# The-Learning-And-Vision-Atelier-LAVA/BUFFER

Measured on AMD Instinct MI355X. Metric: registration pairs/sec, higher is better.
Workload: dtype f32

## Files before the change

buffer_amd/_lib.py:

```python
import ctypes as C
import os

_HERE = os.path.dirname(os.path.abspath(__file__))
LIB_PATH = os.environ.get("BUF_LIB_PATH") or os.path.join(_HERE, "libbuffer_hip.so")

BUF_OK = 0


class BufferHipError(RuntimeError):
    pass


class buf_grid_t(C.Structure):
    _fields_ = [
        ("ws", C.c_void_p), ("ws_bytes", C.c_size_t),
        ("ns", C.c_int), ("nb", C.c_int),
        ("cells_per_elem", C.c_int64),
        ("radius", C.c_float),
        ("supports", C.c_void_p),
        ("desc", C.c_void_p), ("s_off", C.c_void_p), ("table", C.c_void_p),
        ("sorted", C.c_void_p), ("order", C.c_void_p), ("scan_tmp", C.c_void_p),
    ]


# ... 16 lines not shown
    "buf_grid_subsample_ws_bytes": (_sz, [_i, _i, _i64, _i]),
    "buf_grid_subsample_batch": (_i, [_vp, _i, _vp, _i, _f, _i, _vp, _i, _vp, _vp, _vp, _vp, _i64, _vp, _sz, _vp]),
    "buf_fps_ws_bytes": (_sz, [_i, _i]),
    "buf_fps": (_i, [_vp, _i, _i, _i, _vp, _vp, _sz, _vp]),
    "buf_gather": (_i, [_vp, _vp, _i, _i, _i, _i, _vp, _vp]),
    "buf_group": (_i, [_vp, _vp, _i, _i, _i, _i, _i, _vp, _vp]),
    "buf_ball_query": (_i, [_vp, _vp, _i, _i, _i, _f, _i, _vp, _vp]),
    "buf_three_nn": (_i, [_vp, _vp, _i, _i, _i, _vp, _vp, _vp]),
    "buf_select_patches": (_i, [_vp, _vp, _i, _i, _f, _i, _vp, _vp]),
    "buf_select_patches_batched_ws_bytes": (_sz, [_i, _i]),
    "buf_select_patches_batched": (_i, [_vp, _vp, _i, _vp, _i, _f, _i, _vp, _vp, _sz, _vp]),
    "buf_permute_clouds": (_i, [_vp, _vp, _vp, _i, _vp, _vp]),
    "buf_compact_ws_bytes": (_sz, [_i]),
    "buf_compact_greater": (_i, [_vp, _i, _i, _f, _vp, _vp, _vp, _sz, _vp]),
    "buf_knn_ws_bytes": (_sz, [_i, _i, _i]),
    "buf_knn1_ws_bytes": (_sz, [_i, _i, _i]),
    "buf_knn": (_i, [_vp, _vp, _i, _i, _i, _i, _i, _vp, _vp, _vp, _sz, _vp]),
    "buf_fps_ragged": (_i, [_vp, _vp, _i, _i, _vp, _vp, _sz, _vp]),
    "buf_svd3x3_batched": (_i, [_vp, _i, _vp, _vp, _vp, _vp]),
    "buf_vn_gather_block": (_i, [_vp, _vp, _vp, _vp, _i, _i, _i, _i, _i, _i, _f, _vp, _vp, _vp, _vp, _f, _vp, _vp]),
    "buf_vn_gather_pre_ws_bytes": (_sz, [_i, _i]),
    "buf_vn_gather_block_pre": (_i, [_vp, _vp, _vp, _vp, _i, _i, _i, _i, _i, _f, _vp, _vp, _vp, _vp, _f, _vp, _vp, _sz, _vp]),
    "buf_vn_pointwise": (_i, [_vp, _vp, _i, _i, _i, _vp, _i, _i, _i, _vp, _vp, _vp, _vp, _f, _vp, _vp, _vp]),
    "buf_gather_max": (_i, [_vp, _vp, _i, _i, _i, _i, _vp, _vp]),
    "buf_vn_std": (_i, [_vp, _vp, _i, _i, _vp, _vp]),
    "buf_score_head_ws_bytes": (_sz, [_i, _i]),
    "buf_score_head": (_i, [_vp, _i, _vp, _i, _vp, _vp, _vp, _vp, _f, _vp, _vp, _vp, _vp, _f, _vp, _vp, _vp, _vp, _vp, _i, _vp, _vp, _i, _f,
                            _vp, _vp, _sz, _vp]),
    "buf_patch_voxelize_ws_bytes": (_sz, [_i]),
    "buf_patch_voxelize": (_i, [_vp, _vp, _i, _i, _f, _vp, _i, _i, _vp, _f, _i, _vp, _vp, _vp, _vp, _vp, _vp, _vp,
                                _vp, _vp, _sz, _vp]),
    "buf_cylindrical_net_wg": (_i, [_vp, _i, _vp, _vp, _vp, _vp, _vp, _vp, _vp]),
    "buf_cylindrical_net_wg_supports": (_i, [_vp, _vp]),
    "buf_cylindrical_net_split_safe": (_i, [_vp, _i, _vp, _vp, _vp, _vp, _vp, _vp, _vp, _vp, _vp, _vp, _vp, _vp]),
    "buf_cost_volume_net_split_safe": (_i, [_vp, _vp, _i, _vp, _vp, _i, _vp, _vp, _vp, _vp, _vp, _vp, _vp, _vp]),
    "buf_cylindrical_net_split": (_i, [_vp, _i, _vp, _vp, _vp, _vp, _vp, _vp, _vp, _vp]),
    "buf_cylindrical_net_split_head": (_i, [_vp, _i, _vp, _vp, _vp, _vp, _vp, _vp, _vp, _vp, _vp, _vp]),
    "buf_split_gemm_count": (C.c_longlong, [_i, _i, _i, _i]),
    "buf_split_tile_gemm": (_i, [_vp, _i, _i, _i, _i, _vp]),
    "buf_cost_volume_net_split": (_i, [_vp, _vp, _i, _vp, _vp, _vp, _vp, _vp]),
    "buf_cost_volume_net_split_gather": (_i, [_vp, _i, _vp, _vp, _i, _vp, _vp, _vp, _vp, _vp]),
    "buf_split_filter_count": (C.c_longlong, [_i, _i]),
    "buf_split_tile_filters": (_i, [_vp, _i, _i, _vp]),
    "buf_winograd_tile_weights": (_i, [_vp, _i, _i, _vp]),
    "buf_winograd_f24_tile_weights": (_i, [_vp, _i, _i, _vp]),
    "buf_winograd_group": (_i, [_i, _i]),
    "buf_cost_winograd_group": (_i, [_i]),
    "buf_winograd_tile_filters": (_i, [_vp, _i, _i, _i, _i, _vp]),
    "buf_voxel_downsample_ws_bytes": (_sz, [_i, _i64]),
    "buf_voxel_downsample": (_i, [_vp, _vp, _i, _i, C.c_double, _vp, _vp, _vp, _i64, _vp, _sz, _vp]),
    "buf_voxel_downsample_batch_ws_bytes": (_sz, [_i, _i, _i64]),
    "buf_voxel_downsample_batch": (_i, [_vp, _i, _i, _vp, _i, C.c_double, _vp, _vp, _i64, _vp, _sz, _vp]),
    "buf_knn_normals": (_i, [_vp, _i, _vp, _i, _vp, _i, _i, _vp, _i, _vp, _vp, _vp]),
    "buf_icp_ws_bytes": (_sz, [_i, _i, _i, _i]),
    "buf_icp_batched": (_i, [_vp, _vp, _vp, _vp, _vp, _i, _i, _f, _vp, _i, C.c_double, C.c_double, _vp, _vp, _vp, _vp, _vp,
                             _vp, _sz, _vp]),
    "buf_pair_stats_ws_bytes": (_sz, [_i, _i, _i, _i, _i64]),
    "buf_pair_stats": (_i, [_vp, _vp, _i, _vp, _vp, _i, _vp, _f, _i64, _vp, _vp, _vp, _vp, _sz, _vp]),
    "buf_match_metrics": (_i, [_vp, _vp, _vp, _i, _i, _vp, _vp, _f, _f, _f, _vp, _vp, _vp]),
    "buf_row_linear": (_i, [_vp, _i, _i, _i, _vp, _vp, _i, _vp, _vp]),
    "buf_segment_instance_norm_ws_bytes": (_sz, [_i, _i]),
    "buf_segment_instance_norm": (_i, [_vp, _i, _i, _vp, _i, _f, _vp, _vp, _sz, _vp]),
    "buf_descriptor_head": (_i, [_vp, _i, _vp, _vp, _vp, _vp]),
    "buf_cost_volume_net": (_i, [_vp, _vp, _i, _vp, _vp, _vp, _vp]),
    "buf_cost_volume_net_gather": (_i, [_vp, _i, _vp, _vp, _i, _vp, _vp, _vp, _vp]),
    "buf_hypotheses_score": (_i, [_vp, _vp, _vp, _vp, _vp, _i, _i, _f, _vp, _vp, _vp, _vp, _vp, _vp]),
# ... 36 lines not shown
```

buffer_amd/csrc/buffer_hip.hip:

```cpp
#include <stdlib.h>
#include "core.hip"
#include "radius.hip"
#include "icp.hip"
#include "pairstats.hip"
#include "metrics.hip"
#include "subsample.hip"
#include "pointops.hip"
#include "vn.hip"
#include "voxelize.hip"
#include "registration.hip"
#include "convnet.hip"
#include "convnet_h3.hip"
#include "costnet_h3.hip"
#include "preprocess.hip"
#include "convnet_wg.hip"
#include "convnet_w24.hip"
#include "costnet.hip"
#include "split_safe.hip"
```

buffer_amd/csrc/convnet_w24.hip:

```cpp
#include "common.h"

#define W24_WSTRIDE 768
#define W24_SET_F22(CIN) (16 * 128 * (CIN))

__device__ __forceinline__ void w24_tile(int li, int& ty, int& tx)
{
    const bool last = li == 15;
    ty = last ? 3 : li / 5;
    tx = last ? 4 : li - 5 * ty;
}

__device__ __forceinline__ unsigned w24_row_addr(unsigned act_addr, int a, int li, int lk)
{
    int ty, tx;
    w24_tile(li, ty, tx);
    const int row = 2 * ty - 1 + a;
    return act_addr + 4u * (unsigned)(lk * WG_CS + ((row >= 0 && row <= 6) ? row * WG_ROW + 4 * tx : WG_ZERO));
}

struct W24AddrPark { float a[4]; };
__device__ __forceinline__ void w24_park_addresses(const float* act, int li, int lk, W24AddrPark& pk)
{
    const unsigned act_addr = (unsigned)(size_t)(__attribute__((address_space(3))) const float*)act;
#pragma unroll
// ... 58 lines not shown
        const unsigned adv = more ? 4u * WG_KSTEP : 0u;
        __builtin_amdgcn_sched_barrier(0);
#pragma unroll
        for (int s = 0; s < 4; s++) {
            if (s < 2) W24_LOAD(D[s & 1], P0, P1, (s + 2) * WG_KSTEP)
            else {
                if (s == 2) { P0 += adv; P1 += adv; }
                if constexpr (INEXT >= 0) {
                    unsigned q0 = more ? P0 : RA[A1N], q1 = more ? P1 : RA[A2N];
                    W24_LOAD(D[s & 1], q0, q1, (s - 2) * WG_KSTEP)
                } else
                    W24_LOAD(D[s & 1], P0, P1, (s - 2) * WG_KSTEP)
            }
            __builtin_amdgcn_sched_barrier(0);
#pragma unroll
            for (int n = 0; n < 2; n++)
#pragma unroll
                for (int j = 0; j < 6; j++)
                    acc[n][j] = __builtin_amdgcn_mfma_f32_16x16x4f32(W24_U(n, s & 1, j), V[s & 1][j], acc[n][j], 0, 0, 0);
            __builtin_amdgcn_sched_barrier(0);
            W24_XFORM((s + 1) & 1)
#pragma unroll
            for (int n = 0; n < 2; n++) {
                const unsigned o = s < 2 ? wcur + (s + 2) * W24_WSTRIDE : wn + (s - 2) * W24_WSTRIDE;
                W4[n][s & 1] = wg_ldw(rs, o + n * 256, lofs4);
                W2[n][s & 1] = w24_ldw2(rs, o + 512 + n * 128, lofs2);
            }
            __builtin_amdgcn_sched_barrier(0);
        }
    }
#undef W24_XFORM
}

__device__ __forceinline__ void w24_round(unsigned (&RA)[4], __amdgpu_buffer_rsrc_t rs, unsigned wp, unsigned wp_after, unsigned lofs4, unsigned lofs2,
                                          int niter, unsigned pstride, const float* __restrict__ bias_lane, wgf4 (&W4)[2][2], wgf2 (&W2)[2][2],
                                          wgf4 (&Y)[2][2][4])
{
    using std::integral_constant;
    wgf2 D[2][6];
    wgf4 bv[2];
#pragma unroll
    for (int n = 0; n < 2; n++) bv[n] = *reinterpret_cast<const wgf4*>(bias_lane + n * 16);
    wgf4 acc[2][6];
    float zero = 0.f;
    asm volatile("" : "+v"(zero));
#pragma unroll
    for (int n = 0; n < 2; n++)
#pragma unroll
        for (int j = 0; j < 6; j++) acc[n][j] = (wgf4){ zero, zero, zero, zero };
    auto run = [&](auto ic) __attribute__((always_inline)) {
        constexpr int I = decltype(ic)::value;
        constexpr int INEXT = I == 3 ? 0 : I + 1;
        if constexpr (I == 1) {
#pragma unroll
            for (int n = 0; n < 2; n++) acc[n][1] += bv[n];
        }
        constexpr int ICHAIN = (INEXT != 0 && wg_chains(I)) ? INEXT : -1;
        w24_pass<I, wg_chains(I - 1), ICHAIN>(RA, rs, wp + I * pstride, INEXT == 0 ? wp_after : wp + (I + 1) * pstride, lofs4, lofs2, niter, W4, W2, acc, D);
        __builtin_amdgcn_sched_barrier(0);
#pragma unroll
        for (int n = 0; n < 2; n++) {
            wgf4 f[4];
#pragma unroll
            for (int r = 0; r < 4; r++) {
                const float p = acc[n][1][r] + acc[n][2][r], q = acc[n][1][r] - acc[n][2][r];
                const float t = acc[n][3][r] + acc[n][4][r], d = acc[n][3][r] - acc[n][4][r];
                f[0][r] = acc[n][0][r] + p + t;
                f[1][r] = __builtin_fmaf(2.f, d, q);
                f[2][r] = __builtin_fmaf(4.f, t, p);
                f[3][r] = __builtin_fmaf(8.f, d, q) + acc[n][5][r];
            }
#pragma unroll
            for (int v = 0; v < 4; v++) {
                if constexpr (I == 0) Y[n][1][v] = f[v];
                else if constexpr (I == 1) {
#pragma unroll
                    for (int r = 0; r < 4; r++) Y[n][1][v][r] = __builtin_fmaf(2.f, f[v][r], -Y[n][1][v][r]);
                }
                else if constexpr (I == 2) Y[n][0][v] = f[v];
                else Y[n][1][v] -= f[v];
                if constexpr (I == 2) asm volatile("" : "+v"(Y[n][0][v]));
                else asm volatile("" : "+v"(Y[n][1][v]));
            }
        }
    };
    run(integral_constant<int, 0>{});
    run(integral_constant<int, 1>{});
    run(integral_constant<int, 2>{});
    run(integral_constant<int, 3>{});
}

__device__ __forceinline__ void w24_round_direct(unsigned row5, __amdgpu_buffer_rsrc_t rs, unsigned wp, unsigned lofs, int niter, unsigned pstride,
                                                 const float* __restrict__ bias_lane, wgf4 (&W4)[2][2], wgf4 (&Y)[2])
{
    constexpr int wstride = W24_WSTRIDE;
    wgf4 Wr[3][2][2];
#pragma unroll
    for (int n = 0; n < 2; n++)
#pragma unroll
        for (int k = 0; k < 2; k++) {
            Wr[0][n][k] = W4[n][k];
            Wr[1][n][k] = wg_ldw(rs, wp + pstride + n * 256 + k * wstride, lofs);
            Wr[2][n][k] = wg_ldw(rs, wp + 2 * pstride + n * 256 + k * wstride, lofs);
        }
    float X[2][6];
    unsigned pa = row5;
    WG_LOADD(X[0], pa, 0)
    WG_LOADD(X[1], pa, WG_KSTEP)
    wgf4 acc[2][3];
    float zero = 0.f;
    asm volatile("" : "+v"(zero));
#pragma unroll
    for (int n = 0; n < 2; n++) {
        acc[n][0] = (wgf4){ zero, zero, zero, zero };
        acc[n][1] = (wgf4){ zero, zero, zero, zero };
        acc[n][2] = *reinterpret_cast<const wgf4*>(bias_lane + n * 16);
    }
    float G[2][6];
#define W24_TAPS(SLOT)                                                                                    \
    _Pragma("unroll") for (int n = 0; n < 2; n++) {                                                       \
        const wgf4 u0_ = Wr[0][n][SLOT], u1_ = Wr[1][n][SLOT], u2_ = Wr[2][n][SLOT];                      \
        const float d1_ = wg_sub(u1_[1], u2_[1]), d2_ = wg_sub(u1_[2], u2_[2]);                           \
        G[n][0] = u0_[0]; G[n][1] = wg_sub(u0_[1], u0_[2]); G[n][2] = u0_[3];                             \
        G[n][3] = wg_sub(u1_[0], u2_[0]); G[n][4] = wg_sub(d1_, d2_); G[n][5] = wg_sub(u1_[3], u2_[3]);   \
    }
#define W24_RELOAD(SLOT, OFS)                                                                             \
    _Pragma("unroll") for (int n = 0; n < 2; n++)                                                         \
        _Pragma("unroll") for (int blk = 0; blk < 3; blk++) Wr[blk][n][SLOT] = wg_ldw(rs, (OFS) + blk * pstride + n * 256, lofs);
    W24_TAPS(0)
    W24_RELOAD(0, wp + 2 * wstride)
#pragma unroll 1
    for (int it = 0; it < niter; it++) {
        const bool more = it + 1 < niter;
        const unsigned wcur = wp + 4 * it * wstride;
        const unsigned wn = more ? wcur + 4 * wstride : wp;
        const unsigned adv = more ? 4u * WG_KSTEP : 0u;
        __builtin_amdgcn_sched_barrier(0);
#pragma unroll
        for (int s = 0; s < 4; s++) {
#pragma unroll
            for (int b = 0; b < 3; b++)
#pragma unroll
                for (int a = 0; a < 2; a++)
#pragma unroll
                    for (int n = 0; n < 2; n++)
                        acc[n][b] = __builtin_amdgcn_mfma_f32_16x16x4f32(G[n][a * 3 + b], X[s & 1][a * 3 + b], acc[n][b], 0, 0, 0);
            __builtin_amdgcn_sched_barrier(0);
            if (s < 2) WG_LOADD(X[s & 1], pa, (s + 2) * WG_KSTEP)
            else {
// ... 129 lines not shown
__global__ void __launch_bounds__(WG_THREADS, 2) k_cyl_net_w24_rerun(const float* __restrict__ x, CylWgParams P, float* __restrict__ y)
{
    extern __shared__ float lds[];
    if (P.only_if[blockIdx.x] == 0) return;
    cyl_net_w24_body(x, P, y, lds);
}

extern "C" int buf_winograd_f24_tile_weights(const float* w_host, int cout, int cin, float* out_host)
{
    BUF_REQUIRE(w_host && out_host, BUF_EINVAL, "buf_winograd_f24_tile_weights: null argument");
    BUF_REQUIRE(cout > 0 && cin > 0 && cout % 32 == 0 && cin % 4 == 0, BUF_EINVAL, "buf_winograd_f24_tile_weights: widths %d -> %d", cin, cout);
    static const double G2[4][3] = { { 1, 0, 0 }, { .5, .5, .5 }, { .5, -.5, .5 }, { 0, 0, 1 } };
    const double s6 = 1.0 / 6, s12 = 1.0 / 12, s24 = 1.0 / 24;
    const double G4[6][3] = { { .25, 0, 0 }, { -s6, -s6, -s6 }, { -s6, s6, -s6 }, { s24, s12, s6 }, { s24, -s12, s6 }, { 0, 0, 1 } };
    const int k4 = cin / 4;
    for (int o = 0; o < cout; o++)
        for (int c = 0; c < cin; c++) {
            const float* g = w_host + ((size_t)o * cin + c) * 9;
            const int n = o / 16, lane = (c % 4) * 16 + o % 16;
            for (int i = 0; i < 4; i++) {
                float* blk = out_host + (((size_t)(n / 2) * 4 + i) * k4 + c / 4) * W24_WSTRIDE;
                for (int j = 0; j < 6; j++) {
                    double u = 0;
                    for (int a = 0; a < 3; a++)
                        for (int b = 0; b < 3; b++) u += G2[i][a] * (double)g[3 * a + b] * G4[j][b];
                    if (j == 3 || j == 4) blk[512 + (n % 2) * 128 + lane * 2 + (j - 3)] = (float)u;
                    else blk[(n % 2) * 256 + lane * 4 + (j == 5 ? 3 : j)] = (float)u;
                }
            }
        }
    return BUF_OK;
}

static int w24_launch(const float* x, int npatch, CylWgParams P, float* y, void* stream)
{
    for (int l = 0; l < WG_LAYERS; l++) {
        const bool flag = (P.relu[l] & WG_F24_FLAG) != 0;
        BUF_REQUIRE(P.relu[l] >= 0 && P.relu[l] <= (WG_F24_FLAG | 1), BUF_EINVAL, "buf_cylindrical_net_wg: layer %d has relu flags %d", l, P.relu[l]);
        BUF_REQUIRE(flag == (P.cout[l] == 128), BUF_EINVAL,
                    "buf_cylindrical_net_wg: the F(2x4) flag goes on every layer with 128 output channels and on no other (layer %d: %d -> %d, flags %d)",
                    l, P.cin[l], P.cout[l], P.relu[l]);
        if (flag) P.wt[l] += W24_SET_F22(P.cin[l]);
        P.relu[l] &= 1;
    }
    size_t lds = sizeof(float) * WG_BUF;
    static LdsGrant grant, grant_rerun;
    if (int rc = P.only_if ? grant_dynamic_lds((const void*)k_cyl_net_w24_rerun, lds, grant_rerun) : grant_dynamic_lds((const void*)k_cyl_net_w24, lds, grant)) return rc;
    double macs = 0;
    for (int l = 0; l < WG_LAYERS; l++) macs += 9.0 * P.cin[l] * P.cout[l];
    TimedSpan span;
    bool timed = !P.only_if && timing_begin((hipStream_t)stream, &span, 2.0 * 140 * macs * npatch, BUF_TIMED_CYL_NET);
    if (P.only_if) k_cyl_net_w24_rerun<<<npatch, WG_THREADS, lds, (hipStream_t)stream>>>(x, P, y);
    else k_cyl_net_w24<<<npatch, WG_THREADS, lds, (hipStream_t)stream>>>(x, P, y);
    if (timed) timing_end((hipStream_t)stream, &span);
    BUF_LAUNCH_CHECK();
    return BUF_OK;
}
```

buffer_amd/csrc/convnet_wg.hip:

```cpp
#include "common.h"
#include <type_traits>

#define WG_CS 160
#define WG_ROW 22
#define WG_ZERO 154
#define WG_MAXC 128
#define WG_LAYERS 8
#define WG_THREADS 256
#define WG_BUF (WG_MAXC * WG_CS)
#define WG_KSTEP (16 * WG_CS)
#define WG_BLOCKS 16

typedef float wgf4 __attribute__((ext_vector_type(4)));
typedef float wgf2 __attribute__((ext_vector_type(2)));
typedef const __attribute__((address_space(3))) wgf2* wg_lds_f2;

struct CylWgParams {
    const float* wt[WG_LAYERS];
    const float* bias[WG_LAYERS];
    int cin[WG_LAYERS], cout[WG_LAYERS], relu[WG_LAYERS];
    const int* only_if;
#ifdef WG_STAMP
    long long* stamps;
#endif
// ... 588 lines not shown
extern "C" int buf_winograd_tile_weights(const float* w_host, int cout, int cin, float* out_host)
{
    BUF_REQUIRE(cout > 0 && cin > 0 && cout % 16 == 0 && cin % 4 == 0, BUF_EINVAL, "buf_winograd_tile_weights: widths %d -> %d", cin, cout);
    return buf_winograd_tile_filters(w_host, cout, cin, wg_group(cin, cout), WG_BLOCKS / 4, out_host);
}

extern "C" int buf_winograd_group(int cin, int cout) { return wg_group(cin, cout); }

static int wg_check_widths(const int* cin, const int* cout)
{
    for (int l = 0; l < WG_LAYERS; l++) {
        const int ci = cin[l], co = cout[l];
        BUF_REQUIRE(ci > 0 && ci % 16 == 0 && ci <= WG_MAXC && (co == 32 || co == 64 || co == 128), BUF_EINVAL,
                    "buf_cylindrical_net_wg: layer %d has unsupported widths %d -> %d", l, ci, co);
        BUF_REQUIRE(co != 128 || ci % 32 == 0, BUF_EINVAL,
                    "buf_cylindrical_net_wg: layer %d has unsupported widths %d -> %d (128 output channels need Cin %% 32 == 0)", l, ci, co);
        BUF_REQUIRE(co != 32 || (ci % 32 == 0 && ci <= 64), BUF_EINVAL,
                    "buf_cylindrical_net_wg: layer %d has unsupported widths %d -> %d (32 output channels need Cin = 32 or 64)", l, ci, co);
        BUF_REQUIRE(l == 0 || ci == cout[l - 1], BUF_EINVAL, "buf_cylindrical_net_wg: layer %d width mismatch", l);
        BUF_REQUIRE(l == 0 || cout[l - 1] != 32 || co == 32, BUF_EINVAL,
                    "buf_cylindrical_net_wg: layer %d has unsupported widths %d -> %d (only 32-output layers may follow a 32-output layer)", l, ci, co);
    }
    BUF_REQUIRE(cout[WG_LAYERS - 1] == 32, BUF_EINVAL, "buf_cylindrical_net_wg: the last layer must have 32 channels");
    return BUF_OK;
}

extern "C" int buf_cylindrical_net_wg_supports(const int* cin_host, const int* cout_host)
{
    BUF_REQUIRE(cin_host && cout_host, BUF_EINVAL, "buf_cylindrical_net_wg_supports: null argument");
    return wg_check_widths(cin_host, cout_host);
}

#define WG_F24_FLAG BUF_CYL_F24
static inline bool wg_f24_flagged(int relu) { return relu == WG_F24_FLAG || relu == (WG_F24_FLAG | 1); }
static int w24_launch(const float* x, int npatch, CylWgParams P, float* y, void* stream);

static int wg_launch(const float* x, int npatch, const float* const* wt_host, const float* const* bias_host, const int* cin_host,
                     const int* cout_host, const int* relu_host, float* y, const int* only_if, void* stream)
{
    BUF_REQUIRE(npatch >= 0, BUF_EINVAL, "buf_cylindrical_net_wg: npatch=%d", npatch);
    if (npatch == 0) return BUF_OK;
    BUF_REQUIRE(x && y && wt_host && bias_host && cin_host && cout_host && relu_host, BUF_EINVAL, "buf_cylindrical_net_wg: null argument");
    CylWgParams P;
    for (int l = 0; l < WG_LAYERS; l++) {
        P.wt[l] = wt_host[l]; P.bias[l] = bias_host[l];
        P.cin[l] = cin_host[l]; P.cout[l] = cout_host[l]; P.relu[l] = relu_host[l];
        BUF_REQUIRE(P.wt[l] && P.bias[l], BUF_EINVAL, "buf_cylindrical_net_wg: null weights for layer %d", l);
    }
    if (int rc = wg_check_widths(P.cin, P.cout)) return rc;
    P.only_if = only_if;
    for (int l = 0; l < WG_LAYERS; l++)
        if (wg_f24_flagged(relu_host[l])) return w24_launch(x, npatch, P, y, stream);
    size_t lds = sizeof(float) * WG_BUF;
    static LdsGrant grant, grant_rerun;
    if (int rc = only_if ? grant_dynamic_lds((const void*)k_cyl_net_wg_rerun, lds, grant_rerun) : grant_dynamic_lds((const void*)k_cyl_net_wg, lds, grant)) return rc;
    double macs = 0;
    for (int l = 0; l < WG_LAYERS; l++) macs += 9.0 * P.cin[l] * P.cout[l];
    TimedSpan span;
    bool timed = !only_if && timing_begin((hipStream_t)stream, &span, 2.0 * 140 * macs * npatch, BUF_TIMED_CYL_NET);
#ifdef WG_STAMP
    BUF_CHECK_HIP(hipMalloc(&P.stamps, (size_t)npatch * (4 * 20 + 4) * sizeof(long long)));
#endif
    if (only_if) k_cyl_net_wg_rerun<<<npatch, WG_THREADS, lds, (hipStream_t)stream>>>(x, P, y);
    else k_cyl_net_wg<<<npatch, WG_THREADS, lds, (hipStream_t)stream>>>(x, P, y);
    if (timed) timing_end((hipStream_t)stream, &span);
    BUF_LAUNCH_CHECK();
#ifdef WG_STAMP
// ... 35 lines not shown
```

buffer_amd/csrc/core.hip:

```cpp
#include "common.h"
#include <stdarg.h>

static thread_local char g_err[512] = "";

void buf_set_error(const char* fmt, ...)
{
    va_list ap;
    va_start(ap, fmt);
    vsnprintf(g_err, sizeof(g_err), fmt, ap);
    va_end(ap);
}

extern "C" const char* buf_last_error(void) { return g_err; }
extern "C" int buf_version(void) { return 600; }

#include <mutex>
#include <vector>
struct TimedSpan { hipEvent_t a, b; double bytes; int id; };
static std::mutex g_time_mu;
static std::vector<TimedSpan> g_spans;
static int g_timing_on = 0;

extern "C" void buf_timing_enable(int on) { std::lock_guard<std::mutex> l(g_time_mu); g_timing_on = on; }

static bool timing_begin(hipStream_t s, TimedSpan* sp, double bytes, int id = BUF_TIMED_GRID_QUERY)
{
    if (!g_timing_on) return false;
    sp->id = id;
    if (hipEventCreate(&sp->a) != hipSuccess || hipEventCreate(&sp->b) != hipSuccess) return false;
    sp->bytes = bytes;
    (void)hipEventRecord(sp->a, s);
    return true;
}

static void timing_end(hipStream_t s, TimedSpan* sp)
{
    (void)hipEventRecord(sp->b, s);
    std::lock_guard<std::mutex> l(g_time_mu);
    g_spans.push_back(*sp);
}

extern "C" long long buf_timing_collect_kernel(int id, double* total_ms, double* total_work)
{
    std::lock_guard<std::mutex> l(g_time_mu);
    double ms = 0, by = 0;
    long long n = 0;
    std::vector<TimedSpan> keep;
// ... 223 lines not shown
```

buffer_amd/csrc/split_safe.hip:

```cpp
#include "common.h"

extern "C" int buf_cylindrical_net_split_safe(const float* x, int npatch, const void* const* wt_split_host, const float* const* wt_wg_host,
                                              const float* const* bias_host, const int* cin_host, const int* cout_host, const int* relu_host,
                                              const float* head_params, float* y_or_equi, float* desc, int* status_dev, int* flags_ws,
                                              void* stream)
{
    BUF_REQUIRE(npatch >= 0, BUF_EINVAL, "buf_cylindrical_net_split_safe: npatch=%d", npatch);
    if (npatch == 0) return BUF_OK;
    BUF_REQUIRE(x && y_or_equi && flags_ws && wt_split_host && wt_wg_host && bias_host && cin_host && cout_host && relu_host, BUF_EINVAL,
                "buf_cylindrical_net_split_safe: null argument");
    BUF_REQUIRE(!head_params || desc, BUF_EINVAL, "buf_cylindrical_net_split_safe: head without desc");
    if (int rc = buf_cylindrical_net_wg_supports(cin_host, cout_host)) return rc;
    hipStream_t s = (hipStream_t)stream;
    BUF_CHECK_HIP(hipMemsetAsync(flags_ws, 0, sizeof(int) * (size_t)npatch, s));
    int relu_split[WG_LAYERS];
    for (int l = 0; l < WG_LAYERS; l++) relu_split[l] = wg_f24_flagged(relu_host[l]) ? (relu_host[l] & 1) : relu_host[l];
    int rc = h3_launch(x, npatch, wt_split_host, bias_host, cin_host, cout_host, relu_split, head_params ? nullptr : y_or_equi, head_params,
                       desc, head_params ? y_or_equi : nullptr, status_dev, stream, flags_ws);
    if (rc) return rc;
    rc = wg_launch(x, npatch, wt_wg_host, bias_host, cin_host, cout_host, relu_host, y_or_equi, flags_ws, stream);
    if (rc) return rc;
    if (head_params) {
        k_desc_head_masked<<<npatch, DH_THREADS, 0, s>>>(y_or_equi, head_params, desc, y_or_equi, flags_ws);
        BUF_LAUNCH_CHECK();
    }
    return BUF_OK;
}

extern "C" int buf_cost_volume_net_split_safe(const float* s_eq, const float* t_eq, int ele_n, const long long* s_rows, const long long* t_rows,
                                              int m, const void* const* wt_split_host, const float* const* bias_split_host,
                                              const float* const* wt_f32_host, const float* const* bias_f32_host, float* ind_out,
                                              int* status_dev, int* flags_ws, void* stream)
{
    BUF_REQUIRE(m >= 0, BUF_EINVAL, "buf_cost_volume_net_split_safe: m=%d", m);
    if (m == 0) return BUF_OK;
    BUF_REQUIRE(s_eq && t_eq && wt_split_host && bias_split_host && wt_f32_host && bias_f32_host && ind_out && flags_ws, BUF_EINVAL,
                "buf_cost_volume_net_split_safe: null argument");
    BUF_REQUIRE((s_rows == nullptr) == (t_rows == nullptr), BUF_EINVAL, "buf_cost_volume_net_split_safe: one row list without the other");
    BUF_REQUIRE(!s_rows || ele_n == 7, BUF_EINVAL, "buf_cost_volume_net_split_safe: ele_n=%d (the kernels are built for ele_n = 7)", ele_n);
    hipStream_t s = (hipStream_t)stream;
    BUF_CHECK_HIP(hipMemsetAsync(flags_ws, 0, sizeof(int) * (size_t)m, s));
    int rc = cost_net_h3_launch(s_eq, t_eq, m, wt_split_host, bias_split_host, s_rows, t_rows, ele_n, ind_out, status_dev, stream,
                                "buf_cost_volume_net_split_safe", flags_ws);
    if (rc) return rc;
    return cost_net_launch(s_eq, t_eq, m, wt_f32_host, bias_f32_host, s_rows, t_rows, ele_n, ind_out, stream, "buf_cost_volume_net_split_safe", flags_ws);
// ... 2 lines not shown
```

buffer_amd/ops.py:

```python
import ctypes as C
import time
import os
import numpy as np
import torch

from . import _lib
from ._lib import buf_grid_t, check


def _stream():
    return C.c_void_p(torch.cuda.current_stream().cuda_stream)


def _dev(t, dtype, what):
    if not isinstance(t, torch.Tensor) or not t.is_cuda:
        raise _lib.BufferHipError(f"{what}: expected a tensor in device memory (buffer_amd has no CPU path)")
    if t.dtype != dtype:
        t = t.to(dtype)
    return t.contiguous()


def _ptr(t):
    return C.c_void_p(t.data_ptr()) if t is not None else C.c_void_p(0)

# ... 560 lines not shown
    G5 = np.concatenate([G, [[0, 1, 0]]])
    U = np.einsum('ia,ocab,jb->ijoc', G5, np.asarray(w, np.float64), G)
    U = U[:blocks].reshape(blocks, 4, cout // (16 * ng), ng, 16, cin // 4, 4)
    return np.ascontiguousarray(np.transpose(U, (2, 0, 5, 3, 6, 4, 1)), dtype=np.float32).reshape(-1)


def winograd_f24_tile_weights(w):
    cout, cin = w.shape[0], w.shape[1]
    assert cin % 4 == 0 and cout % 32 == 0
    U = winograd_f24_filters(w)
    U = U.reshape(4, 6, cout // 32, 2, 16, cin // 4, 4)
    U = np.transpose(U, (2, 0, 5, 3, 6, 4, 1))
    lead = U.shape[:3]
    wide = U[..., [0, 1, 2, 5]].reshape(*lead, 512)
    narrow = U[..., [3, 4]].reshape(*lead, 256)
    return np.ascontiguousarray(np.concatenate([wide, narrow], axis=-1), dtype=np.float32).reshape(-1)


F24_G2 = np.array([[1, 0, 0], [.5, .5, .5], [.5, -.5, .5], [0, 0, 1]], np.float64)
F24_G4 = np.array([[.25, 0, 0], [-1 / 6, -1 / 6, -1 / 6], [-1 / 6, 1 / 6, -1 / 6], [1 / 24, 1 / 12, 1 / 6], [1 / 24, -1 / 12, 1 / 6], [0, 0, 1]],
                  np.float64)


def winograd_f24_filters(w):
    w64 = np.asarray(w, np.float64)
    U = np.zeros((4, 6) + w64.shape[:2], np.float64)
    for a in range(3):
        for b in range(3):
            U += (F24_G2[:, a][:, None, None, None] * w64[None, None, :, :, a, b]) * F24_G4[:, b][None, :, None, None]
    return U


F24_FLAG = 2


def cyl_layer_filters(w):
    wt = winograd_tile_weights(w)
    if w.shape[0] != 128:
        return wt, 0
    return np.concatenate([wt, winograd_f24_tile_weights(w)]), F24_FLAG


class CylindricalNet:

    def __init__(self, layers, device, f24=True):
        self.wt, self.bias, self.cin, self.cout, self.relu = [], [], [], [], []
        self.entry = "buf_cylindrical_net_wg"
        flags = []
        for w, b, relu in layers:
            cout, cin = w.shape[0], w.shape[1]
            wt, flag = cyl_layer_filters(w) if f24 else (winograd_tile_weights(w), 0)
            flags.append(flag)
            self.wt.append(torch.from_numpy(wt).to(device))
            self.bias.append(torch.from_numpy(np.ascontiguousarray(b, dtype=np.float32)).to(device))
            self.cin.append(cin); self.cout.append(cout); self.relu.append(1 if relu else 0)
        n = len(layers)
        self._wp = (C.c_void_p * n)(*[t.data_ptr() for t in self.wt])
        self._bp = (C.c_void_p * n)(*[t.data_ptr() for t in self.bias])
        self._ci = (C.c_int * n)(*self.cin)
        self._co = (C.c_int * n)(*self.cout)
        self._re = (C.c_int * n)(*[r | f for r, f in zip(self.relu, flags)])

    def __call__(self, x):
        L = _lib.lib()
        x = x.contiguous()
        P = x.shape[0]
        y = torch.empty((P, self.cout[-1], 7, 20), dtype=torch.float32, device=x.device)
        check(L.buf_cylindrical_net_wg(_ptr(x), P, self._wp, self._bp, self._ci, self._co, self._re, _ptr(y), _stream()), self.entry)
        return y


def split_tile_filters(w):
    L = _lib.lib()
    w = np.ascontiguousarray(w, dtype=np.float32)
    cout, cin = w.shape[0], w.shape[1]
    out = np.empty(L.buf_split_filter_count(cout, cin), dtype=np.uint16)
    check(L.buf_split_tile_filters(w.ctypes.data, cout, cin, out.ctypes.data), "buf_split_tile_filters")
    return out


class CylindricalNetSplit:

    def __init__(self, layers, device):
        self.wt, self.bias, self.cin, self.cout, self.relu = [], [], [], [], []
        self.entry = "buf_cylindrical_net_split"
        for w, b, relu in layers:
            cout, cin = w.shape[0], w.shape[1]
            self.wt.append(torch.from_numpy(split_tile_filters(w).view(np.int16)).to(device))
            self.bias.append(torch.from_numpy(np.ascontiguousarray(b, dtype=np.float32)).to(device))
            self.cin.append(cin); self.cout.append(cout); self.relu.append(1 if relu else 0)
        n = len(layers)
        self.status = torch.zeros(1, dtype=torch.int32, device=device)
        self._wp = (C.c_void_p * n)(*[t.data_ptr() for t in self.wt])
        self._bp = (C.c_void_p * n)(*[t.data_ptr() for t in self.bias])
        self._ci = (C.c_int * n)(*self.cin)
        self._co = (C.c_int * n)(*self.cout)
        self._re = (C.c_int * n)(*self.relu)
        self.last_flags = None
        self.safe = n == 8 and _lib.lib().buf_cylindrical_net_wg_supports(self._ci, self._co) == 0 and not os.environ.get('BUF_SPLIT_UNSAFE')
        if self.safe:
            tiled = [cyl_layer_filters(w) for w, _, _ in layers]
            self.wt_wg = [torch.from_numpy(wt).to(device) for wt, _ in tiled]
            self._wwp = (C.c_void_p * n)(*[t.data_ptr() for t in self.wt_wg])
            self._re_safe = (C.c_int * n)(*[r | f for r, (_, f) in zip(self.relu, tiled)])

    def _safe_call(self, x, head):
        L = _lib.lib()
        x = x.contiguous()
        P = x.shape[0]
        out = torch.empty((P, self.cout[-1], 7, 20), dtype=torch.float32, device=x.device)
        desc = torch.empty((P, 32), dtype=torch.float32, device=x.device) if head is not None else None
        self.last_flags = torch.empty((max(P, 1),), dtype=torch.int32, device=x.device)
        check(L.buf_cylindrical_net_split_safe(_ptr(x), P, self._wp, self._wwp, self._bp, self._ci, self._co, self._re_safe,
                                               _ptr(head.params) if head is not None else None, _ptr(out), _ptr(desc), _ptr(self.status),
                                               _ptr(self.last_flags), _stream()), "buf_cylindrical_net_split_safe")
        return (desc, out) if head is not None else out

    def __call__(self, x):
        if self.safe:
            return self._safe_call(x, None)
        L = _lib.lib()
        x = x.contiguous()
        P = x.shape[0]
        y = torch.empty((P, self.cout[-1], 7, 20), dtype=torch.float32, device=x.device)
        check(L.buf_cylindrical_net_split(_ptr(x), P, self._wp, self._bp, self._ci, self._co, self._re, _ptr(y), _ptr(self.status), _stream()),
              self.entry)
        return y

    def with_head(self, x, head):
        if self.safe:
            return self._safe_call(x, head)
        L = _lib.lib()
        x = x.contiguous()
        P = x.shape[0]
# ... 187 lines not shown
```

include/buffer_hip.h:

```cpp
#ifndef BUFFER_HIP_H
#define BUFFER_HIP_H
#include <stddef.h>
#include <stdint.h>
#ifdef __cplusplus
extern "C" {
#endif

#define BUF_OK            0
#define BUF_EINVAL       -1
#define BUF_EHIP         -2
#define BUF_EWORKSPACE   -3
#define BUF_ECAPACITY    -4
#define BUF_ENODEVICE    -5

const char* buf_last_error(void);
int         buf_version(void);
int         buf_device_count(void);
#define BUF_TIMED_GRID_QUERY 0
#define BUF_TIMED_CYL_NET    1
#define BUF_TIMED_COST_NET   2
#define BUF_TIMED_SELECT_PATCHES 3
#define BUF_TIMED_PATCH_VOXELIZE 4
#define BUF_TIMED_FPS            5
#define BUF_TIMED_NN1            6
// ... 76 lines not shown
int     buf_vn_gather_block_pre(const float* q_pts, const float* s_pts, const float* feats, const int* idx,
                                int nq, int ns, int k, int cin, int cout, float scale,
                                const float* wf, const float* wd, const float* bn_scale, const float* bn_shift,
                                float slope, float* out, void* ws, size_t ws_bytes, void* stream);
int     buf_vn_pointwise(const float* a, const int* ind_a, int ind_stride, int na, int ca, const float* b, int cb,
                         int n, int cout, const float* wf, const float* wd, const float* bn_scale,
                         const float* bn_shift, float slope, const float* residual, float* out, void* stream);
int     buf_gather_max(const float* feats, const int* idx, int nq, int ns, int k, int width, float* out, void* stream);
int     buf_row_linear(const float* x, int n, int cin, int cout, const float* w, const float* b, int activation, float* out,
                       void* stream);
size_t  buf_segment_instance_norm_ws_bytes(int nseg, int c);
int     buf_segment_instance_norm(const float* x, int n, int c, const int* lens_host, int nseg, float eps, float* out,
                                  void* ws, size_t ws_bytes, void* stream);
int     buf_vn_std(const float* x, const float* z, int n, int c, float* out, void* stream);
size_t  buf_score_head_ws_bytes(int n, int nseg);
int     buf_score_head(const float* x, int n, const int* lens_host, int nseg,
                       const float* vn1_wf, const float* vn1_wd, const float* vn1_bsc, const float* vn1_bsh, float vn1_slope,
                       const float* vn2_wf, const float* vn2_wd, const float* vn2_bsc, const float* vn2_bsh, float vn2_slope,
                       const float* lin, const float* w0, const float* b0, const float* w1, const float* b1, int c1,
                       const float* w2, const float* b2, int final_activation, float eps, float* out,
                       void* ws, size_t ws_bytes, void* stream);

size_t  buf_patch_voxelize_ws_bytes(int ncentres);
int     buf_patch_voxelize(const float* patches, const float* axis, int npatch, int npts, float des_r,
                           const float* centres, int ncentres, int azi_n, const float* azi_cs, float voxel_r,
                           int nsample, const float* mlp_w_host, const float* mlp_b_host, const float* bn_scale_host,
                           const float* bn_shift_host, float* out_x, float* out_R, float* out_rand, float* out_patches,
                           void* ws, size_t ws_bytes, void* stream);

int     buf_winograd_group(int cin, int cout);
int     buf_winograd_tile_weights(const float* w_host, int cout, int cin, float* out_host);
int     buf_winograd_tile_filters(const float* w_host, int cout, int cin, int ng, int nblk, float* out_host);
#define BUF_CYL_F24 2
int     buf_winograd_f24_tile_weights(const float* w_host, int cout, int cin, float* out_host);
int     buf_cylindrical_net_wg(const float* x, int npatch, const float* const* wt_host, const float* const* bias_host,
                               const int* cin_host, const int* cout_host, const int* relu_host, float* y, void* stream);
int     buf_cylindrical_net_wg_supports(const int* cin_host, const int* cout_host);

long long buf_split_filter_count(int cout, int cin);
int     buf_split_tile_filters(const float* w_host, int cout, int cin, unsigned short* out_host);
int     buf_cylindrical_net_split(const float* x, int npatch, const void* const* wt_host, const float* const* bias_host,
                                  const int* cin_host, const int* cout_host, const int* relu_host, float* y, int* status_dev, void* stream);
int     buf_cylindrical_net_split_head(const float* x, int npatch, const void* const* wt_host, const float* const* bias_host,
                                       const int* cin_host, const int* cout_host, const int* relu_host, const float* head_params,
                                       float* desc, float* equi, int* status_dev, void* stream);

int     buf_cylindrical_net_split_safe(const float* x, int npatch, const void* const* wt_split_host, const float* const* wt_wg_host,
                                       const float* const* bias_host, const int* cin_host, const int* cout_host, const int* relu_host,
                                       const float* head_params, float* y_or_equi, float* desc, int* status_dev, int* flags_ws, void* stream);

int     buf_descriptor_head(const float* y, int npatch, const float* params, float* desc, float* equi, void* stream);

int     buf_cost_winograd_group(int layer);
int     buf_cost_volume_net(const float* s_eq, const float* t_eq, int m, const float* const* wt_host,
                            const float* const* bias_host, float* ind_out, void* stream);
int     buf_cost_volume_net_gather(const float* equi, int ele_n, const long long* s_rows, const long long* t_rows, int m,
                                   const float* const* wt_host, const float* const* bias_host, float* ind_out, void* stream);

long long buf_split_gemm_count(int cout, int cin, int ntaps, int nt);
int     buf_split_tile_gemm(const float* w_host, int cout, int cin, int ntaps, int nt, unsigned short* out_host);
int     buf_cost_volume_net_split(const float* s_eq, const float* t_eq, int m, const void* const* wt_host,
                                  const float* const* bias_host, float* ind_out, int* status_dev, void* stream);
int     buf_cost_volume_net_split_gather(const float* equi, int ele_n, const long long* s_rows, const long long* t_rows, int m,
                                         const void* const* wt_host, const float* const* bias_host, float* ind_out,
                                         int* status_dev, void* stream);
int     buf_cost_volume_net_split_safe(const float* s_eq, const float* t_eq, int ele_n, const long long* s_rows, const long long* t_rows,
// ... 62 lines not shown
```

Measured before the change: 164.2.

## Add K-split F(2x4) Winograd path for 64-output-channel cylindrical conv layers

Adds a new kernel variant that runs 64-output-channel layers (with Cin divisible by 64) using the F(2x4) Winograd tiles, splitting the input-channel reduction across wave halves. Partial sums are parked in AGPRs and exchanged through LDS before the bias, ReLU and store step. Only one half adds the bias. The flag is on by default through the Python wrappers, and flag validation is factored into a shared checker. This aims to speed up the 64-channel layers, which previously used the F(2x2) M-split path, at the cost of an extra LDS exchange, extra barriers and higher register pressure.

```diff
diff --git a/buffer_amd/_lib.py b/buffer_amd/_lib.py
--- a/buffer_amd/_lib.py
+++ b/buffer_amd/_lib.py
@@ -72,6 +72,7 @@
                                 _vp, _vp, _sz, _vp]),
     "buf_cylindrical_net_wg": (_i, [_vp, _i, _vp, _vp, _vp, _vp, _vp, _vp, _vp]),
     "buf_cylindrical_net_wg_supports": (_i, [_vp, _vp]),
+    "buf_cylindrical_net_wg_flags": (_i, [_vp, _vp, _vp]),
     "buf_cylindrical_net_split_safe": (_i, [_vp, _i, _vp, _vp, _vp, _vp, _vp, _vp, _vp, _vp, _vp, _vp, _vp, _vp]),
     "buf_cost_volume_net_split_safe": (_i, [_vp, _vp, _i, _vp, _vp, _i, _vp, _vp, _vp, _vp, _vp, _vp, _vp, _vp]),
     "buf_cylindrical_net_split": (_i, [_vp, _i, _vp, _vp, _vp, _vp, _vp, _vp, _vp, _vp]),
diff --git a/buffer_amd/csrc/buffer_hip.hip b/buffer_amd/csrc/buffer_hip.hip
--- a/buffer_amd/csrc/buffer_hip.hip
+++ b/buffer_amd/csrc/buffer_hip.hip
@@ -15,5 +15,6 @@
 #include "preprocess.hip"
 #include "convnet_wg.hip"
 #include "convnet_w24.hip"
+#include "convnet_w24k.hip"
 #include "costnet.hip"
 #include "split_safe.hip"
diff --git a/buffer_amd/csrc/convnet_w24.hip b/buffer_amd/csrc/convnet_w24.hip
--- a/buffer_amd/csrc/convnet_w24.hip
+++ b/buffer_amd/csrc/convnet_w24.hip
@@ -114,6 +114,7 @@
 #undef W24_XFORM
 }
 
+template <bool NOBIAS = false>
 __device__ __forceinline__ void w24_round(unsigned (&RA)[4], __amdgpu_buffer_rsrc_t rs, unsigned wp, unsigned wp_after, unsigned lofs4, unsigned lofs2,
                                           int niter, unsigned pstride, const float* __restrict__ bias_lane, wgf4 (&W4)[2][2], wgf2 (&W2)[2][2],
                                           wgf4 (&Y)[2][2][4])
@@ -122,7 +123,10 @@
     wgf2 D[2][6];
     wgf4 bv[2];
 #pragma unroll
-    for (int n = 0; n < 2; n++) bv[n] = *reinterpret_cast<const wgf4*>(bias_lane + n * 16);
+    for (int n = 0; n < 2; n++) {
+        if constexpr (NOBIAS) bv[n] = bias_lane ? *reinterpret_cast<const wgf4*>(bias_lane + n * 16) : (wgf4){ 0.f, 0.f, 0.f, 0.f };
+        else bv[n] = *reinterpret_cast<const wgf4*>(bias_lane + n * 16);
+    }
     wgf4 acc[2][6];
     float zero = 0.f;
     asm volatile("" : "+v"(zero));
@@ -172,6 +176,7 @@
     run(integral_constant<int, 3>{});
 }
 
+template <bool NOBIAS = false>
 __device__ __forceinline__ void w24_round_direct(unsigned row5, __amdgpu_buffer_rsrc_t rs, unsigned wp, unsigned lofs, int niter, unsigned pstride,
                                                  const float* __restrict__ bias_lane, wgf4 (&W4)[2][2], wgf4 (&Y)[2])
 {
@@ -196,7 +201,8 @@
     for (int n = 0; n < 2; n++) {
         acc[n][0] = (wgf4){ zero, zero, zero, zero };
         acc[n][1] = (wgf4){ zero, zero, zero, zero };
-        acc[n][2] = *reinterpret_cast<const wgf4*>(bias_lane + n * 16);
+        if constexpr (NOBIAS) acc[n][2] = bias_lane ? *reinterpret_cast<const wgf4*>(bias_lane + n * 16) : (wgf4){ zero, zero, zero, zero };
+        else acc[n][2] = *reinterpret_cast<const wgf4*>(bias_lane + n * 16);
     }
     float G[2][6];
 #define W24_TAPS(SLOT)                                                                                    \
@@ -392,17 +398,41 @@
     return BUF_OK;
 }
 
+static int w24_check_flags(const int* cin, const int* cout, const int* relu)
+{
+    for (int l = 0; l < WG_LAYERS; l++) {
+        BUF_REQUIRE(relu[l] >= 0 && relu[l] <= (BUF_CYL_F24K | WG_F24_FLAG | 1), BUF_EINVAL,
+                    "buf_cylindrical_net_wg: layer %d has the relu word %d (bit 0: ReLU, bits 1 and 2: the F(2x4) flags, nothing above)", l, relu[l]);
+        BUF_REQUIRE(!(relu[l] & BUF_CYL_F24K) || (cout[l] == 64 && cin[l] % 64 == 0), BUF_EINVAL,
+                    "buf_cylindrical_net_wg: the K-split F(2x4) flag (bit 2) goes only on layers with 64 output channels and Cin %% 64 == 0 "
+                    "(layer %d: %d -> %d, flags %d)", l, cin[l], cout[l], relu[l]);
+        BUF_REQUIRE(((relu[l] & WG_F24_FLAG) != 0) == (cout[l] == 128), BUF_EINVAL,
+                    "buf_cylindrical_net_wg: the F(2x4) flag goes on every layer with 128 output channels and on no other (layer %d: %d -> %d, flags %d)",
+                    l, cin[l], cout[l], relu[l]);
+    }
+    return BUF_OK;
+}
+
+extern "C" int buf_cylindrical_net_wg_flags(const int* cin_host, const int* cout_host, const int* relu_host)
+{
+    BUF_REQUIRE(cin_host && cout_host && relu_host, BUF_EINVAL, "buf_cylindrical_net_wg_flags: null argument");
+    if (int rc = wg_check_widths(cin_host, cout_host)) return rc;
+    for (int l = 0; l < WG_LAYERS; l++)
+        if (relu_host[l] >= 2) return w24_check_flags(cin_host, cout_host, relu_host);
+    return BUF_OK;
+}
+
+static int w24k_launch(const float* x, int npatch, CylWgParams P, float* y, void* stream);
 static int w24_launch(const float* x, int npatch, CylWgParams P, float* y, void* stream)
 {
+    if (int rc = w24_check_flags(P.cin, P.cout, P.relu)) return rc;
+    bool ksplit = false;
     for (int l = 0; l < WG_LAYERS; l++) {
-        const bool flag = (P.relu[l] & WG_F24_FLAG) != 0;
-        BUF_REQUIRE(P.relu[l] >= 0 && P.relu[l] <= (WG_F24_FLAG | 1), BUF_EINVAL, "buf_cylindrical_net_wg: layer %d has relu flags %d", l, P.relu[l]);
-        BUF_REQUIRE(flag == (P.cout[l] == 128), BUF_EINVAL,
-                    "buf_cylindrical_net_wg: the F(2x4) flag goes on every layer with 128 output channels and on no other (layer %d: %d -> %d, flags %d)",
-                    l, P.cin[l], P.cout[l], P.relu[l]);
-        if (flag) P.wt[l] += W24_SET_F22(P.cin[l]);
-        P.relu[l] &= 1;
-    }
+        if (P.relu[l] & WG_F24_FLAG) P.wt[l] += W24_SET_F22(P.cin[l]);
+        ksplit |= (P.relu[l] & BUF_CYL_F24K) != 0;
+        P.relu[l] &= ~WG_F24_FLAG;
+    }
+    if (ksplit) return w24k_launch(x, npatch, P, y, stream);
     size_t lds = sizeof(float) * WG_BUF;
     static LdsGrant grant, grant_rerun;
     if (int rc = P.only_if ? grant_dynamic_lds((const void*)k_cyl_net_w24_rerun, lds, grant_rerun) : grant_dynamic_lds((const void*)k_cyl_net_w24, lds, grant)) return rc;
diff --git a/buffer_amd/csrc/convnet_w24k.hip b/buffer_amd/csrc/convnet_w24k.hip
--- /dev/null
+++ b/buffer_amd/csrc/convnet_w24k.hip
@@ -0,0 +1,140 @@
+#include "common.h"
+
+#define W24K_FLAG BUF_CYL_F24K
+#define W24K_XCH_C 64
+#define W24K_XCH_QUADS 9
+
+__device__ __forceinline__ void w24k_unpark(const float (&parked)[4 * W24K_XCH_QUADS], wgf4 (&Q)[W24K_XCH_QUADS])
+{
+#pragma unroll
+    for (int q = 0; q < 4 * W24K_XCH_QUADS; q++) asm volatile("v_accvgpr_read_b32 %0, %1" : "=v"(Q[q >> 2][q & 3]) : "a"(parked[q]));
+}
+
+__device__ __forceinline__ void w24k_layer_ksplit(float* __restrict__ act, const float* __restrict__ wt, const float* __restrict__ bias, int cin, int relu,
+                                                  int w, const WgAddrPark& pk, const W24AddrPark& pk24)
+{
+    act[(threadIdx.x >> 1) * WG_CS + WG_ZERO + 4 + (threadIdx.x & 1)] = 0.f;
+    __syncthreads();
+    int lane = threadIdx.x & (WAVE - 1);
+    asm volatile("" : "+v"(lane));
+    const int lk = lane >> 4;
+    const int pair = w & 1, half = w >> 1;
+    const int k4 = cin >> 2, kn = k4 >> 1;
+    const unsigned kofs = (unsigned)(half * kn) * WG_KSTEP;
+    unsigned RA[4];
+#pragma unroll
+    for (int a = 0; a < 4; a++) {
+        asm volatile("v_accvgpr_read_b32 %0, %1" : "=v"(RA[a]) : "a"(pk24.a[a]));
+        RA[a] += kofs;
+    }
+    const __amdgpu_buffer_rsrc_t rs = wg_weights(wt);
+    const unsigned pstride = (unsigned)(k4 * W24_WSTRIDE);
+    const unsigned wp = (unsigned)pair * 4 * pstride + (unsigned)(half * kn) * W24_WSTRIDE;
+    const unsigned lofs4 = lane * 16, lofs2 = lane * 8;
+    const float* bv = half ? nullptr : bias + (2 * pair) * 16 + lk * 4;
+    wgf4 W4[2][2];
+    wgf2 W2[2][2];
+#pragma unroll
+    for (int n = 0; n < 2; n++)
+#pragma unroll
+        for (int k = 0; k < 2; k++) {
+            W4[n][k] = wg_ldw(rs, wp + k * W24_WSTRIDE + n * 256, lofs4);
+            W2[n][k] = w24_ldw2(rs, wp + k * W24_WSTRIDE + 512 + n * 128, lofs2);
+        }
+    wgf4 Y[2][2][4];
+    float park[2][36];
+    w24_round<true>(RA, rs, wp, wp, lofs4, lofs2, kn >> 2, pstride, bv, W4, W2, Y);
+#pragma unroll
+    for (int n = 0; n < 2; n++)
+#pragma unroll
+        for (int q = 0; q < 32; q++) asm volatile("v_accvgpr_write_b32 %0, %1" : "=a"(park[n][q]) : "v"(Y[n][q >> 4][(q >> 2) & 3][q & 3]));
+    const unsigned row5 = wg_parked(pk, 2, 0) + kofs;
+    int lane_d = threadIdx.x & (WAVE - 1);
+    asm volatile("" : "+v"(lane_d));
+    const float* bvd = half ? nullptr : bias + (2 * pair) * 16 + (lane_d >> 4) * 4;
+    wgf4 Yb[2];
+    w24_round_direct<true>(row5, rs, wp, lofs4, kn >> 2, pstride, bvd, W4, Yb);
+#pragma unroll
+    for (int n = 0; n < 2; n++)
+#pragma unroll
+        for (int q = 0; q < 4; q++) asm volatile("v_accvgpr_write_b32 %0, %1" : "=a"(park[n][32 + q]) : "v"(Yb[n][q]));
+    if (cin > W24K_XCH_C) __syncthreads();
+    int lane_s = threadIdx.x & (WAVE - 1);
+    asm volatile("" : "+v"(lane_s));
+    const int xofs = (W24K_XCH_C + (lane_s >> 2)) * WG_CS + (lane_s & 3) * (4 * W24K_XCH_QUADS);
+    wgf4 Q[W24K_XCH_QUADS];
+    if (half) w24k_unpark(park[0], Q);
+    else w24k_unpark(park[1], Q);
+    wgf4* mine = reinterpret_cast<wgf4*>(act + xofs + 16 * w * WG_CS);
+#pragma unroll
+    for (int q = 0; q < W24K_XCH_QUADS; q++) mine[q] = Q[q];
+    __syncthreads();
+    if (half) w24k_unpark(park[1], Q);
+    else w24k_unpark(park[0], Q);
+    const wgf4* theirs = reinterpret_cast<const wgf4*>(act + xofs + 16 * (w ^ 2) * WG_CS);
+    wgf4 Yk[2][4];
+#pragma unroll
+    for (int q = 0; q < W24K_XCH_QUADS; q++) {
+        Q[q] += theirs[q];
+        if (q < 8) Yk[q >> 2][q & 3] = Q[q];
+    }
+    w24_store_tile(Yk, 2 * pair + half, relu, act, lane_s & 15, lane_s >> 4);
+    wg_store_row6<false>(Q[8], 2 * pair + half, relu, act, nullptr, lane_s & 15, lane_s >> 4);
+}
+
+__device__ __forceinline__ void cyl_net_w24k_body(const float* __restrict__ x, const CylWgParams& P, float* __restrict__ y, float* __restrict__ lds)
+{
+    float* act = lds;
+    const int patch = blockIdx.x;
+    const int w = __builtin_amdgcn_readfirstlane(threadIdx.x / WAVE);
+    wg_load_input(x, P, act, patch);
+    WgAddrPark pk;
+    W24AddrPark pk24;
+    {
+        int lane0 = threadIdx.x & (WAVE - 1);
+        asm volatile("" : "+v"(lane0));
+        wg_park_addresses(act, lane0 & 15, lane0 >> 4, pk);
+        w24_park_addresses(act, lane0 & 15, lane0 >> 4, pk24);
+    }
+#pragma unroll 1
+    for (int l = 0; l < WG_LAYERS; l++) {
+        const int cin = P.cin[l], cout = P.cout[l], relu = P.relu[l] & 1;
+        if (cout == 128) w24_layer_pair(act, P.wt[l], P.bias[l], cin, relu, w, pk, pk24);
+        else if (cout == 64 && (P.relu[l] & W24K_FLAG)) w24k_layer_ksplit(act, P.wt[l], P.bias[l], cin, relu, w, pk, pk24);
+        else if (cout == 64) wg_layer_msplit(act, P.wt[l], P.bias[l], cin, cout, relu, w, pk);
+        else if (l < WG_LAYERS - 1) wg_layer_mksplit<false>(act, nullptr, P.wt[l], P.bias[l], cin, cout, relu, w, pk);
+        else wg_layer_mksplit<true>(act, y + (size_t)patch * cout * 140, P.wt[l], P.bias[l], cin, cout, relu, w, pk);
+        __syncthreads();
+    }
+}
+
+__global__ void __launch_bounds__(WG_THREADS, 2) k_cyl_net_w24k(const float* __restrict__ x, CylWgParams P, float* __restrict__ y)
+{
+    extern __shared__ float lds[];
+    cyl_net_w24k_body(x, P, y, lds);
+}
+
+__global__ void __launch_bounds__(WG_THREADS, 2) k_cyl_net_w24k_rerun(const float* __restrict__ x, CylWgParams P, float* __restrict__ y)
+{
+    extern __shared__ float lds[];
+    if (P.only_if[blockIdx.x] == 0) return;
+    cyl_net_w24k_body(x, P, y, lds);
+}
+
+static int w24k_launch(const float* x, int npatch, CylWgParams P, float* y, void* stream)
+{
+    for (int l = 0; l < WG_LAYERS; l++)
+        if (P.relu[l] & W24K_FLAG) P.wt[l] += WG_BLOCKS * P.cout[l] * P.cin[l];
+    size_t lds = sizeof(float) * WG_BUF;
+    static LdsGrant grant, grant_rerun;
+    if (int rc = P.only_if ? grant_dynamic_lds((const void*)k_cyl_net_w24k_rerun, lds, grant_rerun) : grant_dynamic_lds((const void*)k_cyl_net_w24k, lds, grant)) return rc;
+    double macs = 0;
+    for (int l = 0; l < WG_LAYERS; l++) macs += 9.0 * P.cin[l] * P.cout[l];
+    TimedSpan span;
+    bool timed = !P.only_if && timing_begin((hipStream_t)stream, &span, 2.0 * 140 * macs * npatch, BUF_TIMED_CYL_NET);
+    if (P.only_if) k_cyl_net_w24k_rerun<<<npatch, WG_THREADS, lds, (hipStream_t)stream>>>(x, P, y);
+    else k_cyl_net_w24k<<<npatch, WG_THREADS, lds, (hipStream_t)stream>>>(x, P, y);
+    if (timed) timing_end((hipStream_t)stream, &span);
+    BUF_LAUNCH_CHECK();
+    return BUF_OK;
+}
diff --git a/buffer_amd/csrc/convnet_wg.hip b/buffer_amd/csrc/convnet_wg.hip
--- a/buffer_amd/csrc/convnet_wg.hip
+++ b/buffer_amd/csrc/convnet_wg.hip
@@ -644,7 +644,7 @@
 }
 
 #define WG_F24_FLAG BUF_CYL_F24
-static inline bool wg_f24_flagged(int relu) { return relu == WG_F24_FLAG || relu == (WG_F24_FLAG | 1); }
+static inline bool wg_f24_flagged(int relu) { return relu >= 2; }
 static int w24_launch(const float* x, int npatch, CylWgParams P, float* y, void* stream);
 
 static int wg_launch(const float* x, int npatch, const float* const* wt_host, const float* const* bias_host, const int* cin_host,
diff --git a/buffer_amd/csrc/core.hip b/buffer_amd/csrc/core.hip
--- a/buffer_amd/csrc/core.hip
+++ b/buffer_amd/csrc/core.hip
@@ -12,7 +12,7 @@
 }
 
 extern "C" const char* buf_last_error(void) { return g_err; }
-extern "C" int buf_version(void) { return 600; }
+extern "C" int buf_version(void) { return 610; }
 
 #include <mutex>
 #include <vector>
diff --git a/buffer_amd/csrc/split_safe.hip b/buffer_amd/csrc/split_safe.hip
--- a/buffer_amd/csrc/split_safe.hip
+++ b/buffer_amd/csrc/split_safe.hip
@@ -10,7 +10,7 @@
     BUF_REQUIRE(x && y_or_equi && flags_ws && wt_split_host && wt_wg_host && bias_host && cin_host && cout_host && relu_host, BUF_EINVAL,
                 "buf_cylindrical_net_split_safe: null argument");
     BUF_REQUIRE(!head_params || desc, BUF_EINVAL, "buf_cylindrical_net_split_safe: head without desc");
-    if (int rc = buf_cylindrical_net_wg_supports(cin_host, cout_host)) return rc;
+    if (int rc = buf_cylindrical_net_wg_flags(cin_host, cout_host, relu_host)) return rc;
     hipStream_t s = (hipStream_t)stream;
     BUF_CHECK_HIP(hipMemsetAsync(flags_ws, 0, sizeof(int) * (size_t)npatch, s));
     int relu_split[WG_LAYERS];
diff --git a/buffer_amd/ops.py b/buffer_amd/ops.py
--- a/buffer_amd/ops.py
+++ b/buffer_amd/ops.py
@@ -616,24 +616,30 @@
 
 
 F24_FLAG = 2
-
-
-def cyl_layer_filters(w):
+F24K_FLAG = 4
+
+
+def cyl_layer_filters(w, f24k=True):
     wt = winograd_tile_weights(w)
-    if w.shape[0] != 128:
+    cout, cin = w.shape[0], w.shape[1]
+    if cout == 128:
+        flag = F24_FLAG
+    elif f24k and cout == 64 and cin % 64 == 0:
+        flag = F24K_FLAG
+    else:
         return wt, 0
-    return np.concatenate([wt, winograd_f24_tile_weights(w)]), F24_FLAG
+    return np.concatenate([wt, winograd_f24_tile_weights(w)]), flag
 
 
 class CylindricalNet:
 
-    def __init__(self, layers, device, f24=True):
+    def __init__(self, layers, device, f24=True, f24k=True):
         self.wt, self.bias, self.cin, self.cout, self.relu = [], [], [], [], []
         self.entry = "buf_cylindrical_net_wg"
         flags = []
         for w, b, relu in layers:
             cout, cin = w.shape[0], w.shape[1]
-            wt, flag = cyl_layer_filters(w) if f24 else (winograd_tile_weights(w), 0)
+            wt, flag = cyl_layer_filters(w, f24k) if f24 else (winograd_tile_weights(w), 0)
             flags.append(flag)
             self.wt.append(torch.from_numpy(wt).to(device))
             self.bias.append(torch.from_numpy(np.ascontiguousarray(b, dtype=np.float32)).to(device))
@@ -665,7 +671,7 @@
 
 class CylindricalNetSplit:
 
-    def __init__(self, layers, device):
+    def __init__(self, layers, device, f24k=True):
         self.wt, self.bias, self.cin, self.cout, self.relu = [], [], [], [], []
         self.entry = "buf_cylindrical_net_split"
         for w, b, relu in layers:
@@ -683,7 +689,7 @@
         self.last_flags = None
         self.safe = n == 8 and _lib.lib().buf_cylindrical_net_wg_supports(self._ci, self._co) == 0 and not os.environ.get('BUF_SPLIT_UNSAFE')
         if self.safe:
-            tiled = [cyl_layer_filters(w) for w, _, _ in layers]
+            tiled = [cyl_layer_filters(w, f24k) for w, _, _ in layers]
             self.wt_wg = [torch.from_numpy(wt).to(device) for wt, _ in tiled]
             self._wwp = (C.c_void_p * n)(*[t.data_ptr() for t in self.wt_wg])
             self._re_safe = (C.c_int * n)(*[r | f for r, (_, f) in zip(self.relu, tiled)])
diff --git a/include/buffer_hip.h b/include/buffer_hip.h
--- a/include/buffer_hip.h
+++ b/include/buffer_hip.h
@@ -132,6 +132,8 @@
 int     buf_winograd_tile_weights(const float* w_host, int cout, int cin, float* out_host);
 int     buf_winograd_tile_filters(const float* w_host, int cout, int cin, int ng, int nblk, float* out_host);
 #define BUF_CYL_F24 2
+#define BUF_CYL_F24K 4
+int     buf_cylindrical_net_wg_flags(const int* cin_host, const int* cout_host, const int* relu_host);
 int     buf_winograd_f24_tile_weights(const float* w_host, int cout, int cin, float* out_host);
 int     buf_cylindrical_net_wg(const float* x, int npatch, const float* const* wt_host, const float* const* bias_host,
                                const int* cin_host, const int* cout_host, const int* relu_host, float* y, void* stream);
```

New measurement: 168.4, median of 6. +2.5%, better.
